# HSU-ANT/gstpeaq

Hardware: AMD Instinct MI355X
Metric: 2048-sample stereo ref/test frame-pairs/sec (basic PEAQ, ear model -> MOVs -> ODG); ODG delta vs CPU ref (higher is better)
Workload: dtype f64

## Files before the change

### gstpeaq_amd/csrc/peaq_frontend.hip

```cpp
#include <hip/hip_runtime.h>

#include "peaq_device.h"
#include "peaq_kernels.h"
#include <type_traits>

#include "peaq_wave.h"

namespace peaq {

#ifndef PEAQ_FE_PREFETCH_ITEMS
#define PEAQ_FE_PREFETCH_ITEMS 64
#endif
constexpr int kPrefetchItems = PEAQ_FE_PREFETCH_ITEMS;
constexpr int kUnitDoubles = 1288;
constexpr int kOffPw = 0;
constexpr int kOffScratch = 776;
constexpr int kPwLen = 776;
constexpr int kOffLogTab = 2 * kUnitDoubles;
constexpr int kLogTabDoubles = 2 * kLogTabEntries + 2;
constexpr int kLdsDoubles = 2 * kUnitDoubles + 2 * kLogTabDoubles;
#ifndef PEAQ_FE_WAVES
#define PEAQ_FE_WAVES 3
#endif
constexpr int kWavesPerSimd = PEAQ_FE_WAVES;

__device__ constexpr double kW32re[16] = {1., 0.98078528040323044913, 0.92387953251128675613, 0.83146961230254523708,
                                          0.70710678118654752440, 0.55557023301960222474, 0.38268343236508977173,
                                          0.19509032201612826785, 0., -0.19509032201612826785, -0.38268343236508977173,
                                          -0.55557023301960222474, -0.70710678118654752440, -0.83146961230254523708,
                                          -0.92387953251128675613, -0.98078528040323044913};
__device__ constexpr double kW32im[16] = {-0., -0.19509032201612826785, -0.38268343236508977173, -0.55557023301960222474,
                                          -0.70710678118654752440, -0.83146961230254523708, -0.92387953251128675613,
                                          -0.98078528040323044913, -1., -0.98078528040323044913, -0.92387953251128675613,
                                          -0.83146961230254523708, -0.70710678118654752440, -0.55557023301960222474,
                                          -0.38268343236508977173, -0.19509032201612826785};

__device__ __forceinline__ int pad16(int i) { return i + (i >> 4); }

__device__ __forceinline__ cplx tw_lane(const CommonTables* __restrict__ ct, int e, int lane) {
  const double2 v = *reinterpret_cast<const double2*>(ct->tw_lane[e][lane]);
  return {v.x, v.y};
}
__device__ __forceinline__ cplx csqr(cplx a) { return {a.re * a.re - a.im * a.im, 2. * (a.re * a.im)}; }

template <typename WR, typename RD>
__device__ __forceinline__ void exchange16(cplx (&z)[16], double* buf, WR wr, RD rd) {
#pragma unroll
  for (int r = 0; r < 16; ++r) buf[pad16(wr(r))] = z[r].re;
  wave_lds_fence();
#pragma unroll
  for (int r = 0; r < 16; ++r) z[r].re = buf[pad16(rd(r))];
  wave_lds_fence();
#pragma unroll
  for (int r = 0; r < 16; ++r) buf[pad16(wr(r))] = z[r].im;
  wave_lds_fence();
#pragma unroll
  for (int r = 0; r < 16; ++r) z[r].im = buf[pad16(rd(r))];
  wave_lds_fence();
}

__device__ __forceinline__ void frame_power_spectrum(cplx (&z)[16], double (&p)[16], double* unit, int lane,
                                                     const CommonTables* __restrict__ ct,
                                                     double level_factor) {
  dft16(z);
  exchange16(z, unit, [&](int r) { return 16 * lane + r; }, [&](int r) { return lane + 64 * r; });
  {
    {
      cplx w[9];
      w[1] = tw_lane(ct, 2, lane);
      w[2] = csqr(w[1]);
      w[4] = csqr(w[2]);
      w[8] = csqr(w[4]);
      w[3] = cmul(w[1], w[2]);
      w[5] = cmul(w[4], w[1]);
      w[6] = cmul(w[4], w[2]);
      w[7] = cmul(w[4], w[3]);
#pragma unroll
      for (int r = 1; r < 8; ++r) {
        z[8 + r] = cmul(z[8 + r], cmul(w[8], w[r]));
        z[r] = cmul(z[r], w[r]);
      }
      z[8] = cmul(z[8], w[8]);
    }
    dft16(z);
#ifndef PEAQ_FE_LDS_EXCHANGE2
#pragma unroll
    for (int g = 0; g < 4; ++g) {
      rows_transpose4(z[4 * g].re, z[4 * g + 1].re, z[4 * g + 2].re, z[4 * g + 3].re);
      rows_transpose4(z[4 * g].im, z[4 * g + 1].im, z[4 * g + 2].im, z[4 * g + 3].im);
    }
#pragma unroll
    for (int a2 = 0; a2 < 4; ++a2)
#pragma unroll
      for (int g = a2 + 1; g < 4; ++g) {
        const cplx t = z[4 * a2 + g];
        z[4 * a2 + g] = z[4 * g + a2];
        z[4 * g + a2] = t;
      }
#else
    const int k = lane & 15, j = (lane - k) * 16 + k;
    exchange16(z, unit, [&](int r) { return j + 16 * r; },
               [&](int s) { return lane + 64 * (s & 3) + 256 * (s >> 2); });
#endif
  }
  {
    constexpr double c1 = 0.92387953251128673848, s1 = 0.38268343236508977173, c2 = 0.70710678118654752440;
    const cplx wb = tw_lane(ct, 1, lane);
#pragma unroll
    for (int m = 0; m < 4; ++m) {
      const cplx w1 = m == 0 ? wb : m == 1 ? cmul(wb, {c1, -s1}) : m == 2 ? cmul(wb, {c2, -c2}) : cmul(wb, {s1, -c1});
      const cplx w2 = csqr(w1), w3 = cmul(w2, w1);
      z[m + 4] = cmul(z[m + 4], w1);
      z[m + 8] = cmul(z[m + 8], w2);
      z[m + 12] = cmul(z[m + 12], w3);
      dft4(z[m], z[m + 4], z[m + 8], z[m + 12]);
    }
  }
  wave_lds_fence();
  const cplx wl = tw_lane(ct, 0, lane);
  const int partner = (64 - lane) & 63;
  const double lf4 = 0.25 * level_factor;
#pragma unroll
  for (int q = 0; q < 8; ++q) {
    const int k = lane + 64 * q;
    cplx zm = {__shfl(z[15 - q].re, partner, 64), __shfl(z[15 - q].im, partner, 64)};
    if (lane == 0) zm = z[(16 - q) & 15];
    const cplx e2 = {z[q].re + zm.re, z[q].im - zm.im};
    const cplx o2 = {z[q].im + zm.im, zm.re - z[q].re};
    const cplx wq = {kW32re[q], kW32im[q]};
    const cplx t = cmul(q == 0 ? wl : cmul(wl, wq), o2);
    const cplx xp = cadd(e2, t), xm = csub(e2, t);
    p[q] = (xp.re * xp.re + xp.im * xp.im) * lf4;
    double pm = (xm.re * xm.re + xm.im * xm.im) * lf4;
    int km = 1024 - k;
    if (q == 0 && lane == 0) {
      pm = (z[8].re * z[8].re + z[8].im * z[8].im) * level_factor;
      km = 512;
    }
    p[8 + q] = pm;
    const double2 ew = *reinterpret_cast<const double2*>(ct->ear_w2_pair[q][lane]);
    unit[kOffPw + k] = p[q] * ew.x;
    if (km < kPwLen) unit[kOffPw + km] = pm * ew.y;
  }
  wave_lds_fence();
}

__device__ __forceinline__ int spec_bin(int s, int lane) {
  if (s < 8) return lane + 64 * s;
  if (lane == 0 && s == 8) return 512;
  return 1024 - lane - 64 * (s - 8);
}

struct BandEdge {
  int lo, hi;
  double wlo, whi;
};
__device__ __forceinline__ BandEdge load_band_edge(const BandTables* __restrict__ bt, int b) {
  return {bt->lo[b], bt->hi[b], bt->wlo[b], bt->whi[b]};
}
__device__ __forceinline__ double group_band(const BandEdge& e, const double* sp, int zero) {
  const int lo = e.lo, hi = e.hi;
  double p = e.wlo * sp[lo] + e.whi * sp[hi];
  for (int k0 = lo + 1; k0 < hi; k0 += 8) {
    typedef const __attribute__((address_space(3))) double* lds_cptr;
    const lds_cptr q = (lds_cptr)sp + k0, z = (lds_cptr)sp + zero;
    const int n = hi - k0;
    double v[8];
#pragma unroll
    for (int j = 0; j < 8; ++j) {
      lds_cptr qj = j < n ? q : z - j;
      asm("" : "+v"(qj));
      v[j] = qj[j];
    }
#pragma unroll
    for (int j = 0; j < 8; ++j) p += v[j];
  }
  return p < 1e-12 ? 1e-12 : p;
}

__device__ __forceinline__ int boundary_detect(const float* ax, int n, int lane) {
  const double thr = 200. / 32768;
  double wmax = 0.;
  for (int i = 5 + lane; i < n; i += 64) {
    const double w = (double)ax[i] + (double)ax[i - 1] + (double)ax[i - 2] + (double)ax[i - 3] + (double)ax[i - 4];
    wmax = fmax(wmax, w);
  }
  wmax = wave_max(wmax);
  if (wmax >= thr + 1e-6) return 1;
  if (wmax < thr - 1e-6) return 0;
  int res = 0;
  if (lane == 0) {
    float sum = 0;
    for (int i = 0; i < 5; ++i) sum = (float)((double)sum + (double)ax[i]);
    for (int i = 5; i < n; ++i) {
      sum = (float)((double)sum + ((double)ax[i] - (double)ax[i - 5]));
      if ((double)sum >= thr) {
        res = 1;
        break;
      }
    }
  }
  return __builtin_amdgcn_readfirstlane(res);
}

__device__ __forceinline__ unsigned xcd_remap(unsigned b, unsigned n) {
  const unsigned q = n >> 3, r = n & 7, xcd = b & 7, slot = b >> 3;
  const unsigned base = xcd < r ? xcd * (q + 1) : r * (q + 1) + (xcd - r) * q;
  return base + slot;
}

typedef unsigned int u32x2 __attribute__((ext_vector_type(2)));

struct FrameSrc {
  __amdgpu_buffer_rsrc_t rs;
  int channels, chan;
  __device__ __forceinline__ void set(const float* x, long long s0, long long n_valid, int channels_, int chan_) {
    channels = channels_;
    chan = chan_;
    long long l = n_valid - s0;
    l = l < 0 ? 0 : l > kFrame ? kFrame : l;
    const unsigned long long v = reinterpret_cast<unsigned long long>(x + s0 * channels);
    const unsigned lo = __builtin_amdgcn_readfirstlane((unsigned)v);
    const unsigned hi = __builtin_amdgcn_readfirstlane((unsigned)(v >> 32));
    float* p = reinterpret_cast<float*>(((unsigned long long)hi << 32) | lo);
    rs = __builtin_amdgcn_make_buffer_rsrc(p, 0, __builtin_amdgcn_readfirstlane((int)l * channels * 4), 0x00020000);
  }
  __device__ __forceinline__ int lane_offset(int lane) const { return channels == 1 ? lane * 8 : lane * 16 + chan * 4; }
  __device__ __forceinline__ void load2(int r, int voff, float& x0, float& x1) const {
    if (channels == 1) {
      const u32x2 v = __builtin_amdgcn_raw_buffer_load_b64(rs, voff, r * 512, 0);
      x0 = __uint_as_float(v.x);
      x1 = __uint_as_float(v.y);
    } else {
      x0 = __uint_as_float(__builtin_amdgcn_raw_buffer_load_b32(rs, voff, r * 1024, 0));
      x1 = __uint_as_float(__builtin_amdgcn_raw_buffer_load_b32(rs, voff + 8, r * 1024, 0));
    }
  }
};

#ifdef PEAQ_FE_PROFILE
#define FE_MARK(i)                                                                     \
  do {                                                                                 \
    const unsigned long long now_ = __builtin_readcyclecounter();                      \
    if (a.prof && lane == 0 && (blockIdx.x & 127) == 5) atomicAdd(a.prof + sig * 16 + (i), now_ - prof_t_); \
    prof_t_ = __builtin_readcyclecounter();                                            \
  } while (0)
#else
#define FE_MARK(i) do { } while (0)
#endif

template <int NB>
__global__ __launch_bounds__(128, kWavesPerSimd)
#ifdef PEAQ_FE_NUM_VGPR
__attribute__((amdgpu_num_vgpr(PEAQ_FE_NUM_VGPR)))
#endif
void frontend_kernel(FrontendArgs a) {
  extern __shared__ double lds[];
  __builtin_amdgcn_s_setprio(3);
#ifndef PEAQ_FE_LAZY_KERNARGS
  asm volatile("" ::"s"(a.ref), "s"(a.test), "s"(a.pair_stride), "s"(a.n_ref), "s"(a.n_test), "s"(a.n_uniform_ref),
               "s"(a.n_uniform_test), "s"(a.n_frames), "s"(a.n_frames_uniform), "s"(a.frame_origin), "s"(a.off_ref),
               "s"(a.off_test), "s"(a.channels), "s"(a.frame0), "s"(a.frames_per_launch), "s"(a.fpl_magic), "s"(a.common),
               "s"(a.records), "s"(a.pair_frame0), "s"(gridDim.x));
#endif
  const int lane = threadIdx.x & 63;
  const int sig = __builtin_amdgcn_readfirstlane(threadIdx.x >> 6);
#ifdef PEAQ_FE_PROFILE
  unsigned long long prof_t_ = __builtin_readcyclecounter();
  if (a.prof && lane == 0 && (blockIdx.x & 127) == 5) atomicAdd(a.prof + 32 + sig, 1ull);
#endif
  double* unit = lds + sig * kUnitDoubles;
  double* scratch = unit + kOffScratch;
  const CommonTables* __restrict__ ct = a.common;
  const BandTables* __restrict__ bt = a.bands;

  auto decode = [&](unsigned it, unsigned& pair_, unsigned& fl_) {
    const unsigned t = it >> (a.channels - 1);
    pair_ = a.frames_per_launch == 1 ? t : __umulhi(t, a.fpl_magic);
    fl_ = t - pair_ * a.frames_per_launch;
    return (int)(it & (unsigned)(a.channels - 1));
  };
  const unsigned item = xcd_remap(blockIdx.x, gridDim.x);
  unsigned pair, fl;
  const int chan = decode(item, pair, fl);
  FE_MARK(15);
  const unsigned n_ref = a.n_ref ? a.n_ref[pair] : a.n_uniform_ref;
  const unsigned n_test = a.n_test ? a.n_test[pair] : a.n_uniform_test;
  unsigned frame, frame_origin;
  if (a.pair_frame0) {
    if (fl >= a.pair_nframes[pair]) return;
    frame_origin = a.pair_frame0[pair];
    frame = frame_origin + fl;
  } else {
    frame = a.frame0 + fl;
    frame_origin = a.frame_origin;
    const unsigned n_frames = a.n_frames ? a.n_frames[pair] : a.n_frames_uniform;
    if (frame >= n_frames) return;
  }
  const size_t pair_off = (size_t)pair * a.pair_stride * a.channels;
  FrameSrc src_ref, src_test;
  {
    const long long s0 = (long long)(frame - frame_origin) * kHop;
    src_ref.set(a.ref + pair_off, s0 + a.off_ref, (long long)n_ref, a.channels, chan);
    src_test.set(a.test + pair_off, s0 + a.off_test, (long long)n_test, a.channels, chan);
  }
  const FrameSrc& src = sig ? src_test : src_ref;
  double* __restrict__ rec =
      a.records + ((size_t)(pair * a.frames_per_launch + fl) * a.channels + chan) * kRecDoubles;
  constexpr double kHannA = 0.81649658092772603273;
  constexpr double kHannC[16] = {1.0, 0.923806101034885660186, 0.7068354246185547448714, 0.3821516543455241229047,
                                 -0.0007673650086148258012924, -0.3835694472988822502431, -0.7079202261619581075015,
                                 -0.9243926006499437062869, -0.9999988223018871071366, -0.9232174254904238786877,
                                 -0.7057489581976599840459, -0.3807329612736016723471, 0.002302093218395832312485,
                                 0.3849863367942118830771, 0.7090033602727326108775, 0.9249769229541590372578};
  constexpr double kHannS[16] = {0.0, 0.382860663545790020567, 0.7073780336597309217442, 0.92409962292005024589,
                                 0.99999970557542843387, 0.923512035167290059731, 0.7062923993579444458354,
                                 0.3814424201155840173045, -0.001534729565367423810065, -0.3842780051874341062575,
                                 -0.7084620018059667117941, -0.924685034052046356158, -0.9999973501798961346679,
                                 -0.9229222721777677728372, -0.705205101457706221079, -0.3800232782373413192215};
  const double2 hl0 = *reinterpret_cast<const double2*>(&ct->hann_lane[lane][0]);
  const double2 hl1 = *reinterpret_cast<const double2*>(&ct->hann_lane[lane][2]);
  double* ltab = lds + kOffLogTab + sig * kLogTabDoubles;
  FE_MARK(13);
  cplx z[16];
  float amax = 0.f;
  double energy = 0., hop = 0.;
  {
    const int voff = src.lane_offset(lane);
#pragma unroll
    for (int r = 0; r < 16; ++r) {
      const int n = lane + 64 * r;
      float x0, x1;
      src.load2(r, voff, x0, x1);
      const double w0 = fma(hl0.y, kHannS[r], fma(-hl0.x, kHannC[r], kHannA));
      const double w1 = fma(hl1.y, kHannS[r], fma(-hl1.x, kHannC[r], kHannA));
      z[r] = {w0 * (double)x0, w1 * (double)x1};
      if (r >= 8) {
        energy += (double)(x0 * x0);
        energy += (double)(x1 * x1);
      } else if (sig == 0) {
        hop += (double)(x0 * x0);
        hop += (double)(x1 * x1);
      } else {
        float r0, r1;
        src_ref.load2(r, voff, r0, r1);
        hop += (double)((r0 - x0) * (r0 - x0));
        hop += (double)((r1 - x1) * (r1 - x1));
      }
      amax = fmaxf(amax, n == 0 ? fabsf(x1) : fmaxf(fabsf(x0), fabsf(x1)));
    }
  }
  float pf_keep = 0.f;
  if (chan == 0 && !a.pair_frame0) {
    const unsigned it2 = item + kPrefetchItems;
    if (it2 < gridDim.x) {
      unsigned pair2, fl2;
      decode(it2, pair2, fl2);
      const unsigned n2 = sig ? (a.n_test ? a.n_test[pair2] : a.n_uniform_test) : (a.n_ref ? a.n_ref[pair2] : a.n_uniform_ref);
      const long long s2 = (long long)(a.frame0 + fl2 - a.frame_origin) * kHop + (fl2 == 0 ? 0 : kHop);
      FrameSrc pf;
      pf.set((sig ? a.test : a.ref) + (size_t)pair2 * a.pair_stride * a.channels, s2 + (sig ? a.off_test : a.off_ref),
             (long long)n2, a.channels, 0);
      pf_keep = __uint_as_float(__builtin_amdgcn_raw_buffer_load_b32(pf.rs, lane * 128, 0, 0));
      if (fl2 == 0 && a.channels == 2)
        pf_keep += __uint_as_float(__builtin_amdgcn_raw_buffer_load_b32(pf.rs, (64 + lane) * 128, 0, 0));
    }
  }

  __builtin_amdgcn_s_setprio(0);
#ifdef PEAQ_FE_PROFILE
  asm volatile("s_waitcnt vmcnt(0)" ::: "memory");
#endif
  FE_MARK(14);
  wave_sum2(hop, energy, hop, energy);
  if (lane == 0) rec[sig ? kRecNoiseE : kRecSigE] = hop;
  const int energy_flag = energy >= 8000. / (32768. * 32768.);

  int above = 0;
  if (sig == 0) {
    if (__any((double)amax >= 200. / 32768 + 1e-6)) {
      above = 1;
    } else {
      float* ax = reinterpret_cast<float*>(unit);
      int lane_q = lane;
      asm volatile("" : "+v"(lane_q));
      const int voff_q = src.lane_offset(lane_q);
#pragma unroll
      for (int r = 0; r < 16; ++r) {
        const int n = lane_q + 64 * r;
        float x0, x1;
        src.load2(r, voff_q, x0, x1);
        reinterpret_cast<float2*>(ax)[n] = make_float2(fabsf(x0), fabsf(x1));
      }
      wave_lds_fence();
      above = boundary_detect(ax, kFrame, lane);
      wave_lds_fence();
    }
  }

  if (lane == 0)
    rec[sig ? kRecFlagsTest : kRecFlagsRef] = (double)(above | (energy_flag << 1));

  FE_MARK(0);
  double pspec[16];
  frame_power_spectrum(z, pspec, unit, lane, ct, a.level_factor);

  const int gb1 = lane < (NB + 1) / 2 ? lane : 0, gb2 = lane < (NB + 1) / 2 ? NB - 1 - lane : 0;
  const BandEdge edge1 = load_band_edge(bt, gb1), edge2 = load_band_edge(bt, gb2);
  {
    const double2 t0 = *reinterpret_cast<const double2*>(ct->log_tab[lane]);
    const double2 t1 = *reinterpret_cast<const double2*>(ct->log_tab[64 + lane]);
    const double2 t2 = *reinterpret_cast<const double2*>(ct->log_tab[128]);
    reinterpret_cast<double2*>(ltab)[lane] = t0;
    reinterpret_cast<double2*>(ltab)[64 + lane] = t1;
    if (lane == 0) reinterpret_cast<double2*>(ltab)[128] = t2;
    wave_lds_fence();
  }
  FE_MARK(1);
  constexpr bool kAdvanced = NB == 55;
  int bw_ref = 0, bw_test = 0;
  double* xch = lds + kOffLogTab + 2 * kLogTabEntries;
  double thr = 0.;
  auto top_bin = [&](double level, int limit, bool or_equal) {
    int best = 0;
#pragma unroll
    for (int q = 0; q < 8; ++q) {
      unsigned long long m = __ballot(or_equal ? pspec[q] >= level : pspec[q] > level);
      const int nl = limit - 64 * q;
      m &= nl >= 64 ? ~0ull : nl <= 0 ? 0ull : (1ull << nl) - 1ull;
      if (m) best = max(best, 64 * q + 64 - __builtin_clzll(m));
    }
#pragma unroll
    for (int q = 0; q < 8; ++q) {
      unsigned long long m = __ballot(or_equal ? pspec[8 + q] >= level : pspec[8 + q] > level);
      if (q == 0) {
        if ((m & 1ull) && 512 < limit) best = max(best, 513);
        m &= ~1ull;
      }
      const int lo = 1024 - 64 * q - limit + 1;
      m &= lo >= 64 ? 0ull : lo <= 0 ? ~0ull : ~0ull << lo;
      if (m) best = max(best, 1024 - 64 * q - __builtin_ctzll(m) + 1);
    }
    return best;
  };
  if (!kAdvanced && sig == 1) {
    if (lane >= 1) thr = pspec[8];
    if (lane <= 39) thr = fmax(thr, pspec[9]);
    thr = wave_max(thr);
    if (lane == 0) xch[0] = thr;
  }

  FE_MARK(2);
  const double* pw_ref = lds + kOffPw;
  double* pw_test = lds + kUnitDoubles + kOffPw;
  double* sa = lds + kOffScratch;
  double* sb = lds + kUnitDoubles + kOffScratch;
  int* adv_flag = reinterpret_cast<int*>(lds + kOffLogTab + kLogTabDoubles + 2 * kLogTabEntries);
  auto wait_flag = [&](int i) {
    while (__builtin_amdgcn_readfirstlane(*(volatile int*)(adv_flag + i)) == 0) __builtin_amdgcn_s_sleep(1);
    wave_lds_fence();
  };
  if constexpr (kAdvanced) {
    if (sig == 0 && lane == 0) {
      adv_flag[0] = 0;
      adv_flag[1] = 0;
    }
    __syncthreads();
    if (sig == 1) {
#pragma unroll
      for (int j = 0; j < 8; ++j) {
        const int k = lane + 64 * j;
        const double fr = pw_ref[k], ft = pw_test[k];
        sb[k] = (fr == 0. && ft == 0.) ? 0. : FE_LOG_NONNEG(ft / fr, ltab);
      }
      FE_MARK(8);
      wave_lds_fence();
      {
        constexpr int kSteps = (kPwLen + 63) / 64;
        double r[kSteps], t[kSteps];
#pragma unroll
        for (int i = 0; i < kSteps; ++i) {
          const int k = lane + 64 * i < kPwLen ? lane + 64 * i : 0;
          r[i] = pw_ref[k];
          t[i] = pw_test[k];
        }
        wave_lds_fence();
#pragma unroll
        for (int i = 0; i < kSteps; ++i)
          if (lane + 64 * i < kPwLen) pw_test[lane + 64 * i] = r[i] - 2 * sqrt_pos(r[i] * t[i]) + t[i];
      }
      wave_lds_fence();
      if (lane == 0) adv_flag[1] = 1;
      FE_MARK(10);
    }
  }
  if (!kAdvanced || sig == 0) {
    const double* pw = unit + kOffPw;
    constexpr int kZeroSlot = kOffScratch + 400 - kOffPw;
    if (lane == 0) scratch[400] = 0.;
    wave_lds_fence();
    double* ppx = scratch + 256;
    const int b0 = 2 * lane;
    double c_noise[2], c_lnauc[2], c_gil[2];
#pragma unroll
    for (int s2 = 0; s2 < 2; ++s2) {
      const int b = b0 + s2 < NB ? b0 + s2 : 0;
      c_noise[s2] = bt->internal_noise[b];
      c_lnauc[s2] = bt->ln_aUC[b];
      c_gil[s2] = bt->gIL[b];
    }
    if (lane < (NB + 1) / 2) {
      const int b1 = lane, b2 = NB - 1 - lane;
      ppx[b1] = group_band(edge1, pw, kZeroSlot);
      if (b2 != b1) ppx[b2] = group_band(edge2, pw, kZeroSlot);
    }
    wave_lds_fence();
    if (kAdvanced && lane == 0) adv_flag[0] = 1;
    FE_MARK(3);
    constexpr int kLanes = (NB - 1) / 2;
    double ene[2], ae[2], far[2], back2[2];
#pragma unroll
    for (int s = 0; s < 2; ++s) {
      const int b = b0 + s;
      if (b < NB) {
        const double pp = ppx[b] + c_noise[s];
        const double ln_pp = FE_LOG(pp, ltab);
        const double ln_a = c_lnauc[s] + bt->dz02 * ln_pp;
        const double t = exp_fast(0.2 * ln_a), t2 = t * t;
        const double a_uce = t2 * t2 * t;
        const double g_iu = div_fast(1. - exp_fast((double)(NB - b) * ln_a), 1. - a_uce);
        ae[s] = t2;
        ene[s] = exp_fast(0.4 * (ln_pp - FE_LOG(c_gil[s] + g_iu - 1., ltab)));
        {
          double pw = 1., sq = t2;
#pragma unroll
          for (int e = 2 * kLanes - s; e; e >>= 1) {
            if (e & 1) pw *= sq;
            if (e >> 1) sq *= sq;
          }
          far[s] = ene[s] * pw;
        }
        const double t4 = t2 * t2;
        back2[s] = t4 > 1e-290 ? div_fast(1., t4) : 0.;
      } else {
        ae[s] = 0.;
        ene[s] = 0.;
        far[s] = 0.;
        back2[s] = 0.;
      }
    }
    FE_MARK(4);
    double up0 = 0., up1 = 0.;
    {
      double u = far[0], v = far[1];
#pragma unroll 9
      for (int k = kLanes; k >= 1; --k) {
        up0 += u;
        up0 += v;
        up1 = fma(ae[0], u, up1);
        up1 = fma(ae[1], v, up1);
        up0 = lane_below(up0);
        up1 = lane_below(up1);
        u *= back2[0];
        v *= back2[1];
      }
      up1 = fma(ae[0], ene[0], up1);
    }
    FE_MARK(5);
    double dn0, dn1;
    {
      const double al = bt->aLe;
      const double v = wave_suffix_geometric(ene[0] + al * ene[1], al * al, lane);
      const double nxt = lane_above(v);
      dn0 = v;
      dn1 = ene[1] + al * nxt;
    }
    double root[2];
#pragma unroll
    for (int s = 0; s < 2; ++s) {
      const double e2 = (s ? dn1 : dn0) + (s ? up1 : up0);
      root[s] = b0 + s < NB ? sqrt_pos(sqrt_pos(e2)) : 0.;
    }
    if (b0 < kBandStride)
      *reinterpret_cast<double2*>(rec + (sig ? kRecRootTest : kRecRootRef) + b0) = make_double2(root[0], root[1]);

  }
  FE_MARK(6);
  if constexpr (kAdvanced) {
    if (sig == 0) {
      const BandEdge e1 = load_band_edge(bt, gb1), e2 = load_band_edge(bt, gb2);
      if (lane == 0) xch[0] = 0.;
      wait_flag(1);
      const int zero_at = (int)(xch - pw_test);
      if (lane < (NB + 1) / 2) {
        const int b1 = lane, b2 = NB - 1 - lane;
        rec[kRecNoise + b1] = group_band(e1, pw_test, zero_at);
        if (b2 != b1) rec[kRecNoise + b2] = group_band(e2, pw_test, zero_at);
      } else if (lane < (NB + 1) / 2 + kBandStride - NB) {
        rec[kRecNoise + NB + lane - (NB + 1) / 2] = 0.;
      }
      if (lane == 0) {
        rec[kRecBwRef] = 0.;
        rec[kRecBwTest] = 0.;
      }
    } else {
      wait_flag(0);
    }
    FE_MARK(7);
  } else {
    __syncthreads();
    FE_MARK(7);
    if (sig == 0) {
      bw_ref = top_bin(10. * xch[0], 921, false);
      if (lane == 0) xch[1] = (double)bw_ref;
    }
  }

  if constexpr (!kAdvanced) {
    double* dlog = sa;
#ifndef PEAQ_FE_RATIOS_REF
#define PEAQ_FE_RATIOS_REF 3
#endif
    constexpr int kRefRatios = PEAQ_FE_RATIOS_REF;
#pragma unroll
    for (int j = 0; j < 8 - kRefRatios; ++j) {
      if (sig == 0 && j >= kRefRatios) break;
      const int k = (sig == 0 ? 0 : 64 * kRefRatios) + lane + 64 * j;
      const double fr = pw_ref[k], ft = pw_test[k];
      dlog[k] = (fr == 0. && ft == 0.) ? 0. : FE_LOG_NONNEG(ft / fr, ltab);
    }
  }
  if constexpr (!kAdvanced) {
    FE_MARK(8);
    __syncthreads();
    FE_MARK(9);
  }
  if (!kAdvanced && sig == 1) {
    bw_ref = (int)xch[1];
    if (bw_ref > 346) bw_test = top_bin(3.16227766016838 * thr, bw_ref, true);
  }

  if (!kAdvanced && sig == 1) {
    wave_lds_fence();
    {
      constexpr int kSteps = (kPwLen + 63) / 64;
      double r[kSteps], t[kSteps];
#pragma unroll
      for (int i = 0; i < kSteps; ++i) {
        const int k = lane + 64 * i < kPwLen ? lane + 64 * i : 0;
        r[i] = pw_ref[k];
        t[i] = pw_test[k];
      }
      wave_lds_fence();
#pragma unroll
      for (int i = 0; i < kSteps; ++i)
        if (lane + 64 * i < kPwLen) pw_test[lane + 64 * i] = r[i] - 2 * sqrt_pos(r[i] * t[i]) + t[i];
      if (lane == 0) lds[kOffPw] = 0.;
    }
    wave_lds_fence();
    if (lane < (NB + 1) / 2) {
      const int b1 = lane, b2 = NB - 1 - lane;
      rec[kRecNoise + b1] = group_band(edge1, pw_test, kOffPw - kUnitDoubles);
      if (b2 != b1) rec[kRecNoise + b2] = group_band(edge2, pw_test, kOffPw - kUnitDoubles);
    } else if (lane < (NB + 1) / 2 + kBandStride - NB) {
      rec[kRecNoise + NB + lane - (NB + 1) / 2] = 0.;
    }
    if (lane == 0) {
      rec[kRecBwRef] = (double)bw_ref;
      rec[kRecBwTest] = (double)bw_test;
    }
    FE_MARK(10);
  } else if (kAdvanced ? sig == 1 : sig == 0) {
    double* const sa = kAdvanced ? lds + kOffPw : lds + kOffScratch;
    cplx u[8];
    double g[4], run_in;
    {
      const double* d = kAdvanced ? sb : sa;
#pragma unroll
      for (int r = 0; r < 8; ++r) {
        const double v = d[lane + 64 * r];
        u[r] = {r < 4 ? v : 0., v};
      }
      double tot = 0.;
#pragma unroll
      for (int t = 0; t < 4; ++t) {
        const int j = 4 * lane + t;
        const double hi = d[j + 256], lo = d[j];
        g[t] = hi * hi - lo * lo;
        tot += g[t];
      }
      run_in = wave_prefix_sum(tot, lane) - tot;
    }
    wave_lds_fence();
    auto exchange8 = [&](auto wr, auto swz) {
#pragma unroll
      for (int r = 0; r < 8; ++r) {
        const int i = swz(wr(r));
        sa[i] = u[r].re;
        sb[i] = u[r].im;
      }
      wave_lds_fence();
#pragma unroll
      for (int r = 0; r < 8; ++r) {
        const int i = swz(lane + 64 * r);
        u[r] = {sa[i], sb[i]};
      }
      wave_lds_fence();
    };
    auto twiddle8 = [&](cplx w1) {
      cplx w[8];
      w[1] = w1;
      w[2] = csqr(w[1]);
      w[4] = csqr(w[2]);
      w[3] = cmul(w[1], w[2]);
      w[5] = cmul(w[4], w[1]);
      w[6] = cmul(w[4], w[2]);
      w[7] = cmul(w[4], w[3]);
#pragma unroll
      for (int r = 1; r < 8; ++r) u[r] = cmul(u[r], w[r]);
    };
    dft8(u);
    exchange8([&](int r) { return 8 * lane + r; }, [](int i) { return i ^ ((i >> 4) & 7); });
    {
      const int k = lane & 7;
      twiddle8(tw_lane(ct, 4, lane));
      dft8(u);
      const int j = (lane - k) * 8 + k;
      exchange8([&](int r) { return j + 8 * r; }, [](int i) { return i ^ (((i >> 6) & 1) << 3); });
    }
    const cplx w512 = tw_lane(ct, 3, lane);
    twiddle8(w512);
    dft8(u);
    FE_MARK(10);
    const int partner = (64 - lane) & 63;
    cplx cc[4];
    double c256 = 0.;
#pragma unroll
    for (int r = 0; r < 4; ++r) {
      cplx zm = {__shfl(u[7 - r].re, partner, 64), __shfl(u[7 - r].im, partner, 64)};
      if (lane == 0) zm = u[(8 - r) & 7];
      const cplx a2 = {u[r].re + zm.re, u[r].im - zm.im};
      const cplx b2 = {u[r].im + zm.im, zm.re - u[r].re};
      cc[r] = {b2.re * a2.re + b2.im * a2.im, b2.im * a2.re - b2.re * a2.im};
    }
    if (lane == 0) c256 = (2. * u[4].re) * (2. * u[4].im);
    cplx v[4];
#pragma unroll
    for (int r = 0; r < 4; ++r) {
      cplx cm = {__shfl(cc[3 - r].re, partner, 64), __shfl(cc[3 - r].im, partner, 64)};
      if (lane == 0) cm = r == 0 ? cplx{c256, 0.} : cc[4 - r];
      const cplx e = {cc[r].re + cm.re, cc[r].im - cm.im};
      const cplx od = {cc[r].re - cm.re, cc[r].im + cm.im};
      constexpr double c8 = 0.70710678118654752440;
      const cplx wkf = r == 0 ? w512 : r == 1 ? cmul(w512, {c8, -c8}) : r == 2 ? cmul_mi(w512) : cmul(w512, {-c8, -c8});
      const cplx o = cmul(od, {wkf.re, -wkf.im});
      v[r] = {e.re - o.im, -(e.im + o.re)};
    }
    wave_lds_fence();
    double2* xb = reinterpret_cast<double2*>(sa);
    auto fft256 = [&](cplx (&w)[4]) {
#pragma unroll
      for (int pass = 0; pass < 4; ++pass) {
        const int p = 1 << (2 * pass);
        const int k = lane & (p - 1);
        if (pass > 0) {
          if (pass < 3) {
#pragma unroll
            for (int r = 0; r < 4; ++r) {
              const double2 x = xb[lane + 64 * r];
              w[r] = {x.x, x.y};
            }
          }
          const cplx t1 = tw_lane(ct, 4 + pass, lane), t2 = csqr(t1), t3 = cmul(t2, t1);
          w[1] = cmul(w[1], t1);
          w[2] = cmul(w[2], t2);
          w[3] = cmul(w[3], t3);
        }
        dft4(w[0], w[1], w[2], w[3]);
        if (pass < 2) {
          const int j = (lane - k) * 4 + k;
          wave_lds_fence();
#pragma unroll
          for (int r = 0; r < 4; ++r) xb[j + r * p] = make_double2(w[r].re, w[r].im);
          wave_lds_fence();
        } else if (pass == 2) {
          rows_transpose4(w[0].re, w[1].re, w[2].re, w[3].re);
          rows_transpose4(w[0].im, w[1].im, w[2].im, w[3].im);
        }
      }
    };
    fft256(v);
    wave_lds_fence();
    {
      double2* cb = reinterpret_cast<double2*>(sb);
      constexpr double kScale = 1. / 2048.;
      cb[lane] = make_double2(v[0].re * kScale, -v[0].im * kScale);
      cb[lane + 64] = make_double2(v[1].re * kScale, -v[1].im * kScale);
      double run = run_in;
#pragma unroll
      for (int t = 0; t < 4; ++t) {
        sa[4 * lane + t] = run;
        run += g[t];
      }
    }
    wave_lds_fence();
    FE_MARK(11);
    double c[4], dk[4];
#pragma unroll
    for (int m = 0; m < 4; ++m) {
      c[m] = sb[lane + 64 * m];
      dk[m] = sa[lane + 64 * m];
    }
    const double d0 = read_lane<0>(c[0]);
    double cavg = 0.;
#pragma unroll
    for (int m = 0; m < 4; ++m) {
      c[m] *= rsqrt_pos(d0 * (d0 + dk[m]));
      cavg += c[m];
    }
    cavg = a.cfg.ehs_dc_before_window ? wave_sum(cavg) / 256. : 0.;
    const double* __restrict__ win = a.cfg.centre_ehs_window ? ct->ehs_window_centred : ct->ehs_window;
    cplx w4[4];
#pragma unroll
    for (int m = 0; m < 4; ++m) w4[m] = {(c[m] - cavg) * win[lane + 64 * m], 0.};
    wave_lds_fence();
    fft256(w4);
    if (!a.cfg.ehs_dc_before_window && lane == 0) w4[0].re = 0.;
    const double s0 = w4[0].re * w4[0].re + w4[0].im * w4[0].im;
    const double s1 = w4[1].re * w4[1].re + w4[1].im * w4[1].im;
    const double s2 = w4[2].re * w4[2].re + w4[2].im * w4[2].im;
    const double s0_up = lane_below(s0), s1_up = lane_below(s1);
    const double s0_last = read_lane<63>(s0), s1_last = read_lane<63>(s1);
    const double prev0 = s0_up;
    const double prev1 = lane == 0 ? s0_last : s1_up;
    double best = 0.;
    if (lane >= 1 && s0 > prev0) best = s0;
    if (s1 > prev1 && s1 > best) best = s1;
    if (lane == 0 && s2 > s1_last && s2 > best) best = s2;
    best = wave_max(best);
    if (lane == 0) rec[kRecEhs] = best;
    FE_MARK(12);
  }
  if (pf_keep == 123456.789f) rec[kRecScalars + 15] = 1.;
}

hipError_t launch_frontend(int bands, const FrontendArgs& a, unsigned n_pairs, hipStream_t stream) {
  const unsigned grid = n_pairs * a.frames_per_launch * a.channels;
  if (grid == 0) return hipSuccess;
  if ((unsigned long long)n_pairs * a.frames_per_launch * a.channels >= (1ull << 26)) return hipErrorInvalidValue;
  FrontendArgs args = a;
  args.fpl_magic = (unsigned)(((1ull << 32) + a.frames_per_launch - 1) / a.frames_per_launch);
  if (a.frames_per_launch > 1) {
    const unsigned long long err = (unsigned long long)args.fpl_magic * a.frames_per_launch - (1ull << 32);
    const unsigned long long t_max = (unsigned long long)n_pairs * a.frames_per_launch - 1;
    if (err && t_max >= ((1ull << 32) + err - 1) / err) return hipErrorInvalidValue;
  }
#ifndef PEAQ_FE_LDS_PAD
#define PEAQ_FE_LDS_PAD 0
#endif
  const size_t lds = kLdsDoubles * sizeof(double) + PEAQ_FE_LDS_PAD;
  if (bands == 109)
    hipLaunchKernelGGL(frontend_kernel<109>, dim3(grid), dim3(128), lds, stream, args);
  else if (bands == 55)
    hipLaunchKernelGGL(frontend_kernel<55>, dim3(grid), dim3(128), lds, stream, args);
  else
    return hipErrorInvalidValue;
  return hipGetLastError();
}

}
```

Before: 29.76 million.

## Shrink basic front-end LDS footprint to fit more workgroups per CU

Re-lays out the basic-version shared memory per template: smaller per-wave units, a single shared log table, the test wave's scratch overlapping the power-spectrum buffer, and static LDS sizing. It raises the occupancy target to four waves per SIMD, parks one power-spectrum slot in LDS to free registers, and precomputes the test wave's bandwidth ballot masks before the barrier. It also replaces __shfl with ds_bpermute lane reads and switches the advanced flags to acquire/release atomics. The cost is more LDS round-trips (the split re/im exchange, parked slots) and tighter aliasing that could introduce races.

```diff
diff --git a/gstpeaq_amd/csrc/peaq_frontend.hip b/gstpeaq_amd/csrc/peaq_frontend.hip
--- a/gstpeaq_amd/csrc/peaq_frontend.hip
+++ b/gstpeaq_amd/csrc/peaq_frontend.hip
@@ -12,17 +12,30 @@
 #define PEAQ_FE_PREFETCH_ITEMS 64
 #endif
 constexpr int kPrefetchItems = PEAQ_FE_PREFETCH_ITEMS;
-constexpr int kUnitDoubles = 1288;
-constexpr int kOffPw = 0;
-constexpr int kOffScratch = 776;
 constexpr int kPwLen = 776;
-constexpr int kOffLogTab = 2 * kUnitDoubles;
 constexpr int kLogTabDoubles = 2 * kLogTabEntries + 2;
-constexpr int kLdsDoubles = 2 * kUnitDoubles + 2 * kLogTabDoubles;
+
+template <int NB>
+struct FeLds {
+  static constexpr bool kBasic = NB != 55;
+  static constexpr int kUnit = kBasic ? 1088 : 1288;
+  static constexpr int kPwTest = kBasic ? kUnit - kPwLen : 0;
+  static constexpr int kScratchRef = kPwLen;
+  static constexpr int kScratchTest = kBasic ? 0 : kPwLen;
+  static constexpr int kScratchLen = kBasic ? kUnit - kPwLen : 512;
+  static constexpr int kLogTab = 2 * kUnit;
+  static constexpr int kMasks = kLogTab + kLogTabDoubles;
+  static constexpr int kDoubles = kLogTab + (kBasic ? kLogTabDoubles + 16 : 2 * kLogTabDoubles);
+};
+constexpr int kParked = 1;
+static_assert(8 * FeLds<109>::kDoubles <= 160 * 1024 / 8, "eight workgroups of the basic front end per CU");
+static_assert(FeLds<109>::kUnit >= 1088 && FeLds<109>::kScratchLen >= 128 + 64 * kParked, "exchange buffer; ppx, parked slots");
 #ifndef PEAQ_FE_WAVES
-#define PEAQ_FE_WAVES 3
-#endif
-constexpr int kWavesPerSimd = PEAQ_FE_WAVES;
+#define PEAQ_FE_WAVES 4
+#endif
+#ifndef PEAQ_FE_WAVES_ADV
+#define PEAQ_FE_WAVES_ADV 3
+#endif
 
 __device__ constexpr double kW32re[16] = {1., 0.98078528040323044913, 0.92387953251128675613, 0.83146961230254523708,
                                           0.70710678118654752440, 0.55557023301960222474, 0.38268343236508977173,
@@ -37,6 +50,11 @@
 
 __device__ __forceinline__ int pad16(int i) { return i + (i >> 4); }
 
+__device__ __forceinline__ double lane_read(double v, int src) {
+  const int a = src << 2;
+  return __hiloint2double(__builtin_amdgcn_ds_bpermute(a, __double2hiint(v)), __builtin_amdgcn_ds_bpermute(a, __double2loint(v)));
+}
+
 __device__ __forceinline__ cplx tw_lane(const CommonTables* __restrict__ ct, int e, int lane) {
   const double2 v = *reinterpret_cast<const double2*>(ct->tw_lane[e][lane]);
   return {v.x, v.y};
@@ -59,8 +77,8 @@
   wave_lds_fence();
 }
 
-__device__ __forceinline__ void frame_power_spectrum(cplx (&z)[16], double (&p)[16], double* unit, int lane,
-                                                     const CommonTables* __restrict__ ct,
+__device__ __forceinline__ void frame_power_spectrum(cplx (&z)[16], double (&p)[16], double* unit, double* pw, double* park,
+                                                     int lane, const CommonTables* __restrict__ ct,
                                                      double level_factor) {
   dft16(z);
   exchange16(z, unit, [&](int r) { return 16 * lane + r; }, [&](int r) { return lane + 64 * r; });
@@ -123,24 +141,28 @@
 #pragma unroll
   for (int q = 0; q < 8; ++q) {
     const int k = lane + 64 * q;
-    cplx zm = {__shfl(z[15 - q].re, partner, 64), __shfl(z[15 - q].im, partner, 64)};
+    cplx zm = {lane_read(z[15 - q].re, partner), lane_read(z[15 - q].im, partner)};
     if (lane == 0) zm = z[(16 - q) & 15];
     const cplx e2 = {z[q].re + zm.re, z[q].im - zm.im};
     const cplx o2 = {z[q].im + zm.im, zm.re - z[q].re};
     const cplx wq = {kW32re[q], kW32im[q]};
     const cplx t = cmul(q == 0 ? wl : cmul(wl, wq), o2);
     const cplx xp = cadd(e2, t), xm = csub(e2, t);
-    p[q] = (xp.re * xp.re + xp.im * xp.im) * lf4;
+    const double pp = (xp.re * xp.re + xp.im * xp.im) * lf4;
     double pm = (xm.re * xm.re + xm.im * xm.im) * lf4;
     int km = 1024 - k;
     if (q == 0 && lane == 0) {
       pm = (z[8].re * z[8].re + z[8].im * z[8].im) * level_factor;
       km = 512;
     }
+    if (park && q < kParked)
+      park[64 * q + lane] = pp;
+    else
+      p[q] = pp;
     p[8 + q] = pm;
     const double2 ew = *reinterpret_cast<const double2*>(ct->ear_w2_pair[q][lane]);
-    unit[kOffPw + k] = p[q] * ew.x;
-    if (km < kPwLen) unit[kOffPw + km] = pm * ew.y;
+    pw[k] = pp * ew.x;
+    if (km < kPwLen) pw[km] = pm * ew.y;
   }
   wave_lds_fence();
 }
@@ -250,12 +272,13 @@
 #endif
 
 template <int NB>
-__global__ __launch_bounds__(128, kWavesPerSimd)
+__global__ __launch_bounds__(128, NB == 55 ? PEAQ_FE_WAVES_ADV : PEAQ_FE_WAVES)
 #ifdef PEAQ_FE_NUM_VGPR
 __attribute__((amdgpu_num_vgpr(PEAQ_FE_NUM_VGPR)))
 #endif
 void frontend_kernel(FrontendArgs a) {
-  extern __shared__ double lds[];
+  using L = FeLds<NB>;
+  __shared__ __attribute__((aligned(16))) double lds[L::kDoubles];
   __builtin_amdgcn_s_setprio(3);
 #ifndef PEAQ_FE_LAZY_KERNARGS
   asm volatile("" ::"s"(a.ref), "s"(a.test), "s"(a.pair_stride), "s"(a.n_ref), "s"(a.n_test), "s"(a.n_uniform_ref),
@@ -263,14 +286,15 @@
                "s"(a.off_test), "s"(a.channels), "s"(a.frame0), "s"(a.frames_per_launch), "s"(a.fpl_magic), "s"(a.common),
                "s"(a.records), "s"(a.pair_frame0), "s"(gridDim.x));
 #endif
-  const int lane = threadIdx.x & 63;
+  int lane = threadIdx.x & 63;
   const int sig = __builtin_amdgcn_readfirstlane(threadIdx.x >> 6);
 #ifdef PEAQ_FE_PROFILE
   unsigned long long prof_t_ = __builtin_readcyclecounter();
   if (a.prof && lane == 0 && (blockIdx.x & 127) == 5) atomicAdd(a.prof + 32 + sig, 1ull);
 #endif
-  double* unit = lds + sig * kUnitDoubles;
-  double* scratch = unit + kOffScratch;
+  double* unit = lds + sig * L::kUnit;
+  double* scratch = unit + (sig ? L::kScratchTest : L::kScratchRef);
+  double* pw_own = unit + (sig ? L::kPwTest : 0);
   const CommonTables* __restrict__ ct = a.common;
   const BandTables* __restrict__ bt = a.bands;
 
@@ -320,7 +344,7 @@
                                  -0.9229222721777677728372, -0.705205101457706221079, -0.3800232782373413192215};
   const double2 hl0 = *reinterpret_cast<const double2*>(&ct->hann_lane[lane][0]);
   const double2 hl1 = *reinterpret_cast<const double2*>(&ct->hann_lane[lane][2]);
-  double* ltab = lds + kOffLogTab + sig * kLogTabDoubles;
+  double* ltab = lds + L::kLogTab + (L::kBasic ? 0 : sig * kLogTabDoubles);
   FE_MARK(13);
   cplx z[16];
   float amax = 0.f;
@@ -402,12 +426,13 @@
     rec[sig ? kRecFlagsTest : kRecFlagsRef] = (double)(above | (energy_flag << 1));
 
   FE_MARK(0);
+  asm volatile("" : "+v"(lane));
   double pspec[16];
-  frame_power_spectrum(z, pspec, unit, lane, ct, a.level_factor);
-
-  const int gb1 = lane < (NB + 1) / 2 ? lane : 0, gb2 = lane < (NB + 1) / 2 ? NB - 1 - lane : 0;
-  const BandEdge edge1 = load_band_edge(bt, gb1), edge2 = load_band_edge(bt, gb2);
-  {
+  double* const park = L::kBasic ? scratch + 128 : nullptr;
+  frame_power_spectrum(z, pspec, unit, pw_own, park, lane, ct, a.level_factor);
+  asm volatile("" : "+v"(lane));
+
+  auto fill_log_table = [&] {
     const double2 t0 = *reinterpret_cast<const double2*>(ct->log_tab[lane]);
     const double2 t1 = *reinterpret_cast<const double2*>(ct->log_tab[64 + lane]);
     const double2 t2 = *reinterpret_cast<const double2*>(ct->log_tab[128]);
@@ -415,24 +440,30 @@
     reinterpret_cast<double2*>(ltab)[64 + lane] = t1;
     if (lane == 0) reinterpret_cast<double2*>(ltab)[128] = t2;
     wave_lds_fence();
-  }
+  };
+  if constexpr (!L::kBasic) fill_log_table();
   FE_MARK(1);
   constexpr bool kAdvanced = NB == 55;
   int bw_ref = 0, bw_test = 0;
-  double* xch = lds + kOffLogTab + 2 * kLogTabEntries;
+  double* xch = lds + L::kLogTab + 2 * kLogTabEntries;
+  unsigned long long* test_masks = reinterpret_cast<unsigned long long*>(lds + L::kMasks);
   double thr = 0.;
-  auto top_bin = [&](double level, int limit, bool or_equal) {
+  auto slot_mask = [&](int s, double level, bool or_equal) -> unsigned long long {
+    const double v = s < kParked ? park[64 * s + lane] : pspec[s];
+    return __ballot(or_equal ? v >= level : v > level);
+  };
+  auto top_bin = [&](auto mask, int limit) {
     int best = 0;
 #pragma unroll
     for (int q = 0; q < 8; ++q) {
-      unsigned long long m = __ballot(or_equal ? pspec[q] >= level : pspec[q] > level);
+      unsigned long long m = mask(q);
       const int nl = limit - 64 * q;
       m &= nl >= 64 ? ~0ull : nl <= 0 ? 0ull : (1ull << nl) - 1ull;
       if (m) best = max(best, 64 * q + 64 - __builtin_clzll(m));
     }
 #pragma unroll
     for (int q = 0; q < 8; ++q) {
-      unsigned long long m = __ballot(or_equal ? pspec[8 + q] >= level : pspec[8 + q] > level);
+      unsigned long long m = mask(8 + q);
       if (q == 0) {
         if ((m & 1ull) && 512 < limit) best = max(best, 513);
         m &= ~1ull;
@@ -448,17 +479,35 @@
     if (lane <= 39) thr = fmax(thr, pspec[9]);
     thr = wave_max(thr);
     if (lane == 0) xch[0] = thr;
-  }
-
+#pragma unroll
+    for (int s = 0; s < 16; ++s) {
+      const unsigned long long m = slot_mask(s, 3.16227766016838 * thr, true);
+      if (lane == 0) test_masks[s] = m;
+    }
+    fill_log_table();
+  }
   FE_MARK(2);
-  const double* pw_ref = lds + kOffPw;
-  double* pw_test = lds + kUnitDoubles + kOffPw;
-  double* sa = lds + kOffScratch;
-  double* sb = lds + kUnitDoubles + kOffScratch;
-  int* adv_flag = reinterpret_cast<int*>(lds + kOffLogTab + kLogTabDoubles + 2 * kLogTabEntries);
+  if constexpr (!kAdvanced) {
+    __syncthreads();
+    FE_MARK(7);
+    if (sig == 0) {
+      bw_ref = top_bin([&](int s) { return slot_mask(s, 10. * xch[0], false); }, 921);
+      if (lane == 0) xch[1] = (double)bw_ref;
+    }
+  }
+  const int gb1 = lane < (NB + 1) / 2 ? lane : 0, gb2 = lane < (NB + 1) / 2 ? NB - 1 - lane : 0;
+  const BandEdge edge1 = load_band_edge(bt, gb1), edge2 = load_band_edge(bt, gb2);
+  const double* pw_ref = lds;
+  double* pw_test = lds + L::kUnit + L::kPwTest;
+  double* sa = lds + L::kScratchRef;
+  double* sb = lds + L::kUnit + L::kScratchTest;
+  int* adv_flag = reinterpret_cast<int*>(lds + L::kLogTab + kLogTabDoubles + 2 * kLogTabEntries);
   auto wait_flag = [&](int i) {
-    while (__builtin_amdgcn_readfirstlane(*(volatile int*)(adv_flag + i)) == 0) __builtin_amdgcn_s_sleep(1);
-    wave_lds_fence();
+    while (__builtin_amdgcn_readfirstlane(__hip_atomic_load(adv_flag + i, __ATOMIC_ACQUIRE, __HIP_MEMORY_SCOPE_WORKGROUP)) == 0)
+      __builtin_amdgcn_s_sleep(1);
+  };
+  auto set_flag = [&](int i) {
+    if (lane == 0) __hip_atomic_store(adv_flag + i, 1, __ATOMIC_RELEASE, __HIP_MEMORY_SCOPE_WORKGROUP);
   };
   if constexpr (kAdvanced) {
     if (sig == 0 && lane == 0) {
@@ -490,16 +539,16 @@
           if (lane + 64 * i < kPwLen) pw_test[lane + 64 * i] = r[i] - 2 * sqrt_pos(r[i] * t[i]) + t[i];
       }
       wave_lds_fence();
-      if (lane == 0) adv_flag[1] = 1;
+      set_flag(1);
       FE_MARK(10);
     }
   }
   if (!kAdvanced || sig == 0) {
-    const double* pw = unit + kOffPw;
-    constexpr int kZeroSlot = kOffScratch + 400 - kOffPw;
-    if (lane == 0) scratch[400] = 0.;
+    const double* pw = pw_own;
+    const int zero_slot = (int)(scratch + 120 - pw);
+    if (lane == 0) scratch[120] = 0.;
     wave_lds_fence();
-    double* ppx = scratch + 256;
+    double* ppx = scratch;
     const int b0 = 2 * lane;
     double c_noise[2], c_lnauc[2], c_gil[2];
 #pragma unroll
@@ -511,11 +560,11 @@
     }
     if (lane < (NB + 1) / 2) {
       const int b1 = lane, b2 = NB - 1 - lane;
-      ppx[b1] = group_band(edge1, pw, kZeroSlot);
-      if (b2 != b1) ppx[b2] = group_band(edge2, pw, kZeroSlot);
+      ppx[b1] = group_band(edge1, pw, zero_slot);
+      if (b2 != b1) ppx[b2] = group_band(edge2, pw, zero_slot);
     }
     wave_lds_fence();
-    if (kAdvanced && lane == 0) adv_flag[0] = 1;
+    if (kAdvanced) set_flag(0);
     FE_MARK(3);
     constexpr int kLanes = (NB - 1) / 2;
     double ene[2], ae[2], far[2], back2[2];
@@ -607,13 +656,6 @@
       wait_flag(0);
     }
     FE_MARK(7);
-  } else {
-    __syncthreads();
-    FE_MARK(7);
-    if (sig == 0) {
-      bw_ref = top_bin(10. * xch[0], 921, false);
-      if (lane == 0) xch[1] = (double)bw_ref;
-    }
   }
 
   if constexpr (!kAdvanced) {
@@ -622,6 +664,7 @@
 #define PEAQ_FE_RATIOS_REF 3
 #endif
     constexpr int kRefRatios = PEAQ_FE_RATIOS_REF;
+    static_assert(128 + 64 * kParked <= 64 * kRefRatios, "log ratios of the test wave over the parked slots");
 #pragma unroll
     for (int j = 0; j < 8 - kRefRatios; ++j) {
       if (sig == 0 && j >= kRefRatios) break;
@@ -637,7 +680,12 @@
   }
   if (!kAdvanced && sig == 1) {
     bw_ref = (int)xch[1];
-    if (bw_ref > 346) bw_test = top_bin(3.16227766016838 * thr, bw_ref, true);
+    if (bw_ref > 346)
+      bw_test = top_bin([&](int s) {
+        const unsigned long long m = test_masks[s];
+        return ((unsigned long long)__builtin_amdgcn_readfirstlane((unsigned)(m >> 32)) << 32) |
+               (unsigned)__builtin_amdgcn_readfirstlane((unsigned)m);
+      }, bw_ref);
   }
 
   if (!kAdvanced && sig == 1) {
@@ -655,13 +703,13 @@
 #pragma unroll
       for (int i = 0; i < kSteps; ++i)
         if (lane + 64 * i < kPwLen) pw_test[lane + 64 * i] = r[i] - 2 * sqrt_pos(r[i] * t[i]) + t[i];
-      if (lane == 0) lds[kOffPw] = 0.;
+      if (lane == 0) lds[0] = 0.;
     }
     wave_lds_fence();
     if (lane < (NB + 1) / 2) {
       const int b1 = lane, b2 = NB - 1 - lane;
-      rec[kRecNoise + b1] = group_band(edge1, pw_test, kOffPw - kUnitDoubles);
-      if (b2 != b1) rec[kRecNoise + b2] = group_band(edge2, pw_test, kOffPw - kUnitDoubles);
+      rec[kRecNoise + b1] = group_band(edge1, pw_test, (int)(lds - pw_test));
+      if (b2 != b1) rec[kRecNoise + b2] = group_band(edge2, pw_test, (int)(lds - pw_test));
     } else if (lane < (NB + 1) / 2 + kBandStride - NB) {
       rec[kRecNoise + NB + lane - (NB + 1) / 2] = 0.;
     }
@@ -671,7 +719,7 @@
     }
     FE_MARK(10);
   } else if (kAdvanced ? sig == 1 : sig == 0) {
-    double* const sa = kAdvanced ? lds + kOffPw : lds + kOffScratch;
+    double* const sa = kAdvanced ? lds : lds + L::kScratchRef;
     cplx u[8];
     double g[4], run_in;
     {
@@ -693,17 +741,31 @@
     }
     wave_lds_fence();
     auto exchange8 = [&](auto wr, auto swz) {
-#pragma unroll
-      for (int r = 0; r < 8; ++r) {
-        const int i = swz(wr(r));
-        sa[i] = u[r].re;
-        sb[i] = u[r].im;
-      }
-      wave_lds_fence();
-#pragma unroll
-      for (int r = 0; r < 8; ++r) {
-        const int i = swz(lane + 64 * r);
-        u[r] = {sa[i], sb[i]};
+      if constexpr (kAdvanced) {
+#pragma unroll
+        for (int r = 0; r < 8; ++r) {
+          const int i = swz(wr(r));
+          sa[i] = u[r].re;
+          sb[i] = u[r].im;
+        }
+        wave_lds_fence();
+#pragma unroll
+        for (int r = 0; r < 8; ++r) {
+          const int i = swz(lane + 64 * r);
+          u[r] = {sa[i], sb[i]};
+        }
+      } else {
+#pragma unroll
+        for (int r = 0; r < 8; ++r) sa[swz(wr(r))] = u[r].re;
+        wave_lds_fence();
+#pragma unroll
+        for (int r = 0; r < 8; ++r) u[r].re = sa[swz(lane + 64 * r)];
+        wave_lds_fence();
+#pragma unroll
+        for (int r = 0; r < 8; ++r) sa[swz(wr(r))] = u[r].im;
+        wave_lds_fence();
+#pragma unroll
+        for (int r = 0; r < 8; ++r) u[r].im = sa[swz(lane + 64 * r)];
       }
       wave_lds_fence();
     };
@@ -737,7 +799,7 @@
     double c256 = 0.;
 #pragma unroll
     for (int r = 0; r < 4; ++r) {
-      cplx zm = {__shfl(u[7 - r].re, partner, 64), __shfl(u[7 - r].im, partner, 64)};
+      cplx zm = {lane_read(u[7 - r].re, partner), lane_read(u[7 - r].im, partner)};
       if (lane == 0) zm = u[(8 - r) & 7];
       const cplx a2 = {u[r].re + zm.re, u[r].im - zm.im};
       const cplx b2 = {u[r].im + zm.im, zm.re - u[r].re};
@@ -747,7 +809,7 @@
     cplx v[4];
 #pragma unroll
     for (int r = 0; r < 4; ++r) {
-      cplx cm = {__shfl(cc[3 - r].re, partner, 64), __shfl(cc[3 - r].im, partner, 64)};
+      cplx cm = {lane_read(cc[3 - r].re, partner), lane_read(cc[3 - r].im, partner)};
       if (lane == 0) cm = r == 0 ? cplx{c256, 0.} : cc[4 - r];
       const cplx e = {cc[r].re + cm.re, cc[r].im - cm.im};
       const cplx od = {cc[r].re - cm.re, cc[r].im + cm.im};
@@ -791,8 +853,9 @@
     };
     fft256(v);
     wave_lds_fence();
+    double* const sc = kAdvanced ? sb : sa + 256;
     {
-      double2* cb = reinterpret_cast<double2*>(sb);
+      double2* cb = reinterpret_cast<double2*>(sc);
       constexpr double kScale = 1. / 2048.;
       cb[lane] = make_double2(v[0].re * kScale, -v[0].im * kScale);
       cb[lane + 64] = make_double2(v[1].re * kScale, -v[1].im * kScale);
@@ -808,7 +871,7 @@
     double c[4], dk[4];
 #pragma unroll
     for (int m = 0; m < 4; ++m) {
-      c[m] = sb[lane + 64 * m];
+      c[m] = sc[lane + 64 * m];
       dk[m] = sa[lane + 64 * m];
     }
     const double d0 = read_lane<0>(c[0]);
@@ -858,7 +921,7 @@
 #ifndef PEAQ_FE_LDS_PAD
 #define PEAQ_FE_LDS_PAD 0
 #endif
-  const size_t lds = kLdsDoubles * sizeof(double) + PEAQ_FE_LDS_PAD;
+  const size_t lds = PEAQ_FE_LDS_PAD;
   if (bands == 109)
     hipLaunchKernelGGL(frontend_kernel<109>, dim3(grid), dim3(128), lds, stream, args);
   else if (bands == 55)
```

New measurement: 29.56 million, median of 2. Within noise of the previous version (-0.7%).
